# Whisper-6/DynamicTreeAttn

Measured on AMD Instinct MI355X. Metric: tree-attn fwd+bwd tokens/sec, Qwen3-0.6B tau2-16k tries, higher is better.
Workload: dtype bf16

## Files before the change

### dynamictreeattn_amd/csrc/tree_attn.hip

```cpp
#include <hip/hip_runtime.h>
#include <stdint.h>
#include <type_traits>
#include "dta_common.h"
#include "dta_device.h"

#if defined(DTA_STAMP) && DTA_STAMP
__device__ unsigned long long* dta_stamp_buf = nullptr;
extern "C" int dta_debug_set_stamp_buffer(void* p) { return hipMemcpyToSymbol(HIP_SYMBOL(dta_stamp_buf), &p, sizeof(p)) == hipSuccess ? 0 : -4; }
#define DTA_STAMP_DECL unsigned long long st_prev_, st_sum_[6] = {0, 0, 0, 0, 0, 0}; unsigned long long st_tiles_ = 0; \
  __builtin_amdgcn_sched_barrier(0); asm volatile("s_memtime %0\n\ts_waitcnt lgkmcnt(0)" : "=s"(st_prev_) :: "memory"); __builtin_amdgcn_sched_barrier(0);
#define DTA_STAMP_AT(K) { unsigned long long t_; __builtin_amdgcn_sched_barrier(0); asm volatile("s_memtime %0\n\ts_waitcnt lgkmcnt(0)" : "=s"(t_) :: "memory"); \
  __builtin_amdgcn_sched_barrier(0); st_sum_[K] += t_ - st_prev_; st_prev_ = t_; }
#define DTA_STAMP_TILE ++st_tiles_;
#define DTA_STAMP_STORE if (dta_stamp_buf && lane == 0) { unsigned long long* o_ = dta_stamp_buf + ((size_t)blockIdx.x * 8 + wave) * 8; \
  for (int k_ = 0; k_ < 6; ++k_) o_[k_] = st_sum_[k_]; o_[6] = st_tiles_; o_[7] = (unsigned long long)__builtin_amdgcn_s_getreg(0xF804) ; }
#else
#define DTA_STAMP_DECL
#define DTA_STAMP_AT(K)
#define DTA_STAMP_TILE
#define DTA_STAMP_STORE
#endif

namespace {

struct AttnParams {
  const void *q, *k, *v, *o, *dout;
  void *out, *dq, *dk, *dv;
  float *lse_w; const float* lse_r; float* delta;
  const int32_t *subtree_end, *run_ptr, *runs, *ktile_qend;
  const int32_t *dkv_units, *dkv_splits; float* dkv_ws;
  int32_t Tq, Tk, q_offset, Hq, Hkv, group;
  int32_t hgroups, head0;
  int64_t q_st, q_sh, kv_st, kv_sh, v_st, v_sh, o_st, o_sh, dq_st, dq_sh, dkv_st, dkv_sh;
  float scale; int32_t accumulate; int32_t ktile;
};
struct AttnParamsW : AttnParams { const int32_t* win_lo; int32_t window; };
struct AttnParamsC : AttnParams { float softcap; };
struct AttnParamsWC : AttnParamsW { float softcap; };
template <bool WIN, bool CAP = false> using AttnP = typename std::conditional<CAP, typename std::conditional<WIN, AttnParamsWC, AttnParamsC>::type,
                                                                              typename std::conditional<WIN, AttnParamsW, AttnParams>::type>::type;

__device__ __forceinline__ int swz64(int row) { return ((row & 2) << 1) | ((row >> 2) & 3); }
template <int D> __device__ __forceinline__ int img_off_d(int row, int ch) {
  if constexpr (D == 128) return row * 256 + ((ch ^ (((row & 3) << 2) | ((row >> 2) & 3))) << 4);
  else { static_assert(D == 64, "head_dim 64 or 128"); return row * 128 + ((ch ^ swz64(row)) << 4); }
}
template <int D> constexpr int tile_bytes() { return 64 * 2 * D; }

template <class V8, int D> __device__ __forceinline__ V8 row_frag(const char* img, int row, int ch) {
  return *reinterpret_cast<const V8*>(img + img_off_d<D>(row, ch));
}

template <class V8, int D> __device__ __forceinline__ V8 tr_frag(const char* img, int R0, int mb, int lane) {
  const int G = lane >> 4, hh = lane >> 5, i = lane & 15, qd = i >> 2, p = i & 3;
  const int ch = 4 * mb + 2 * (G & 1) + (p >> 1);
  const int ra = R0 + 4 * hh + qd;
  s16x4 lo = tr_read(img + img_off_d<D>(ra, ch) + 8 * (p & 1));
  s16x4 hi = tr_read(img + img_off_d<D>(ra + 8, ch) + 8 * (p & 1));
  s16x8 both = {lo[0], lo[1], lo[2], lo[3], hi[0], hi[1], hi[2], hi[3]};
  return __builtin_bit_cast(V8, both);
}

template <int DT> __device__ __forceinline__ typename Ty<DT>::v8 pack_half(const f32x16& x, int s2) {
  typename Ty<DT>::v8 r;
#pragma unroll
  for (int j = 0; j < 8; ++j) r[j] = (typename Ty<DT>::e)x[8 * s2 + j];
  return r;
}

__device__ __forceinline__ float fast_exp2(float x) { return __builtin_amdgcn_exp2f(x); }

#define DTA_CAP_CONSTANTS                                                                                  \
  const float c = (CAP ? cap_of(p) : p.scale) * LOG2E;                                                     \
  [[maybe_unused]] const float kcap = CAP ? 2.f * LOG2E * p.scale / cap_of(p) : 0.f;
template <class P> __device__ __forceinline__ float cap_of(const P& p) {
  if constexpr (std::is_base_of<AttnParamsC, P>::value || std::is_base_of<AttnParamsWC, P>::value) return p.softcap; else return 0.f;
}

struct TileIter {
  const int32_t* runs; int ri, re;
  int k0, kend, flag;
  int diag_first_q;
  __device__ __forceinline__ bool load_run() {
    while (ri < re) {
      k0 = __builtin_amdgcn_readfirstlane(runs[4 * ri]); kend = __builtin_amdgcn_readfirstlane(runs[4 * ri + 1]);
      flag = __builtin_amdgcn_readfirstlane(runs[4 * ri + 2]);
      if (k0 < kend) return true;
      ++ri;
    }
    return false;
  }
  __device__ __forceinline__ bool advance() {
    k0 += 64;
    if (k0 < kend) return true;
    if (runs == nullptr) return false;
    ++ri;
    return load_run();
  }
  __device__ __forceinline__ bool masked() const {
    if (runs == nullptr) return (k0 + 63 > diag_first_q) || (k0 + 64 > kend);
    return flag != 0 || (k0 + 64 > kend);
  }
};

#ifndef DTA_FWD_THR
#define DTA_FWD_THR 4.0f
#endif
constexpr float FWD_THR = DTA_FWD_THR;
constexpr int SE_BYTES = 256;

__device__ __forceinline__ float max3(float a, float b, float c) { return fmaxf(fmaxf(a, b), c); }
__device__ __forceinline__ float half_max(float x) {
  const unsigned u = __float_as_uint(x);
  const auto r = __builtin_amdgcn_permlane32_swap(u, u, false, false);
  return fmaxf(__uint_as_float(r[0]), __uint_as_float(r[1]));
}

template <int D> struct FragOffsT { int row[D / 16]; int tr[D / 16]; };
template <int D> __device__ __forceinline__ FragOffsT<D> frag_offsets(int lane) {
  FragOffsT<D> o;
  const int r = lane & 31, h = lane >> 5;
#pragma unroll
  for (int s = 0; s < D / 16; ++s) o.row[s] = img_off_d<D>(r, 2 * s + h);
  const int G = lane >> 4, i = lane & 15, qd = i >> 2, pp = i & 3;
#pragma unroll
  for (int mb = 0; mb < D / 32; ++mb) {
    const int ch = 4 * mb + 2 * (G & 1) + (pp >> 1);
    o.tr[mb] = img_off_d<D>(4 * h + qd, ch) + 8 * (pp & 1);
    o.tr[D / 32 + mb] = img_off_d<D>(4 * h + qd + 8, ch) + 8 * (pp & 1);
  }
  return o;
}
template <class V8> __device__ __forceinline__ V8 tr_pair(const char* lo_p, const char* hi_p) {
  s16x4 lo = tr_read(lo_p);
  s16x4 hi = tr_read(hi_p);
  s16x8 both = {lo[0], lo[1], lo[2], lo[3], hi[0], hi[1], hi[2], hi[3]};
  return __builtin_bit_cast(V8, both);
}
template <class V8, int D> __device__ __forceinline__ V8 tr_frag_o(const char* img_r0, const FragOffsT<D>& o, int mb) {
  s16x4 lo = tr_read(img_r0 + o.tr[mb]);
  s16x4 hi = tr_read(img_r0 + o.tr[D / 32 + mb]);
  s16x8 both = {lo[0], lo[1], lo[2], lo[3], hi[0], hi[1], hi[2], hi[3]};
  return __builtin_bit_cast(V8, both);
}

__device__ __forceinline__ uint32_t lds_addr(const void* p) {
  return (uint32_t)(uintptr_t)(__attribute__((address_space(3))) const char*)(p);
}
__device__ __forceinline__ void dma_pair2(uint32_t oa0, uint32_t oa1, const void* ba, uint32_t ob0, uint32_t ob1, const void* bb, uint32_t lds) {
  asm volatile(
      "s_nop 4\n\t"
      "s_mov_b32 m0, %6\n\t"
      "s_nop 0\n\t"
      "global_load_lds_dwordx4 %0, %4\n\t"
      "s_add_u32 m0, %6, 0x4000\n\t"
      "s_nop 0\n\t"
      "global_load_lds_dwordx4 %2, %5\n\t"
      "s_add_u32 m0, %6, 0x400\n\t"
      "s_nop 0\n\t"
      "global_load_lds_dwordx4 %1, %4\n\t"
      "s_add_u32 m0, %6, 0x4400\n\t"
// ... 39 lines not shown
      else reinterpret_cast<int*>(base_ + 2 * tile_bytes<DH>())[lane] = 0x7fffffff; }                     \
    const char* kb_ = reinterpret_cast<const char*>(kbase) + (int64_t)k0_ * p.kv_st * (int64_t)sizeof(e);  \
    const char* vb_ = reinterpret_cast<const char*>(vbase) + (int64_t)k0_ * p.v_st * (int64_t)sizeof(e);   \
    uint32_t ok_[DTA_KV_PPW(NW)], ov_[DTA_KV_PPW(NW)];                                                     \
    _Pragma("unroll") for (int i_ = 0; i_ < DTA_KV_PPW(NW); ++i_) { ok_[i_] = voff_k[i_]; ov_[i_] = voff_v[i_]; } \
    if (k0_ + 64 > p.Tk) {                          \
      _Pragma("unroll") for (int i_ = 0; i_ < DTA_KV_PPW(NW); ++i_) {                                      \
        const int row_ = DTA_KV_ROW(NW, i_);                                                               \
        const int rr_ = k0_ + row_ < p.Tk ? row_ : p.Tk - 1 - k0_;                                         \
        ok_[i_] = dma_src_off_d<DH>(rr_, row_, lane, p.kv_st, sizeof(e)); ov_[i_] = dma_src_off_d<DH>(rr_, row_, lane, p.v_st, sizeof(e)); } } \
    if constexpr (DH == 128) {                                                                             \
      _Pragma("unroll") for (int i_ = 0; i_ < DTA_KV_PPW(NW); i_ += 2)                                     \
        dma_pair2(ok_[i_], ok_[i_ + 1], kb_, ov_[i_], ov_[i_ + 1], vb_, lds_addr(base_ + (wave * DTA_KV_PPW(NW) + i_) * 1024)); \
    } else {                                                                                               \
      _Pragma("unroll") for (int i_ = 0; i_ < DTA_KV_PPW(NW); ++i_)                                        \
        dma_one2<tile_bytes<DH>()>(ok_[i_], kb_, ov_[i_], vb_, lds_addr(base_ + (wave * DTA_KV_PPW(NW) + i_) * 1024)); } }

#ifndef DTA_V_PRELOAD_N
#define DTA_V_PRELOAD_N 4
#endif
#if DTA_V_PRELOAD_N
#define DTA_V_PRELOAD v8 vpre_[DTA_V_PRELOAD_N]; _Pragma("unroll") for (int i_ = 0; i_ < DTA_V_PRELOAD_N; ++i_) { vpre_[i_] = tr_frag_o<v8>(Vs + 32 * DH * (i_ / (DH / 32)), offs, i_ % (DH / 32)); asm volatile("" : "+v"(vpre_[i_])); }
#define DTA_V_FRAG(S4, DB) (((DH / 32) * (S4) + (DB) < DTA_V_PRELOAD_N) ? vpre_[(DH / 32) * (S4) + (DB) < DTA_V_PRELOAD_N ? (DH / 32) * (S4) + (DB) : 0] : tr_frag_o<v8>(Vs + 32 * DH * (S4), offs, (DB)))
#else
#define DTA_V_PRELOAD
#define DTA_V_FRAG(S4, DB) tr_frag_o<v8>(Vs + 32 * DH * (S4), offs, (DB))
#endif

#ifndef DTA_SCORE_ORDER
#define DTA_SCORE_ORDER 1
#endif
#if DTA_SCORE_ORDER
#define DTA_SCORE_MFMAS                                                                                    \
    { v8 ka_ = *reinterpret_cast<const v8*>(Ks + offs.row[0]), kb2_ = *reinterpret_cast<const v8*>(Ks + 64 * DH + offs.row[0]); \
      _Pragma("unroll") for (int s = 0; s < DH / 16; ++s) {                                                \
        v8 na_ = ka_, nb_ = kb2_;                                                                          \
        if (s < DH / 16 - 1) { na_ = *reinterpret_cast<const v8*>(Ks + offs.row[s + 1]); nb_ = *reinterpret_cast<const v8*>(Ks + 64 * DH + offs.row[s + 1]); } \
        X[0] = T::mma(ka_, qf[s], X[0]); X[1] = T::mma(kb2_, qf[s], X[1]);                                 \
        ka_ = na_; kb2_ = nb_;                                                                             \
      } }
#else
#define DTA_SCORE_MFMAS                                                                                    \
    _Pragma("unroll") for (int kb = 0; kb < 2; ++kb)                                                       \
      _Pragma("unroll") for (int s = 0; s < DH / 16; ++s)                                                  \
        X[kb] = T::mma(*reinterpret_cast<const v8*>(Ks + 64 * DH * kb + offs.row[s]), qf[s], X[kb]);
#endif

template <int DT, int HPB, int DH, bool WIN, bool CAP>
__global__ __launch_bounds__(256 * HPB, 2) void tree_attn_fwd_kernel(AttnP<WIN, CAP> p) {
  using T = Ty<DT>; using e = typename T::e; using v8 = typename T::v8; using v4 = typename T::v4;
  constexpr int TB = tile_bytes<DH>(), NKS = DH / 16, NDB = DH / 32;
  constexpr int NW = 4 * HPB, BUF = 2 * TB + SE_BYTES;
  __shared__ __attribute__((aligned(16))) char smem[2 * BUF];

  const int tid = threadIdx.x, lane = tid & 63, r = lane & 31, h = lane >> 5;
  const int wave = __builtin_amdgcn_readfirstlane(tid >> 6);
  const int hb = wave >> 2, rw = wave & 3;
  const int bid = blockIdx.x;
  const int hgroups = p.hgroups;
  const int kvh = bid % p.Hkv; const int rest = bid / p.Hkv; const int hgb = rest % hgroups;
  const int nqt = (p.Tq + DTA_QTILE - 1) / DTA_QTILE;
  const int qt = nqt - 1 - rest / hgroups;
  const int hq = kvh * p.group + p.head0 + hgb * HPB + hb;
  const int q0 = qt * DTA_QTILE;
  const int qrow = q0 + rw * 32 + r;
  const int qrow_c = qrow < p.Tq ? qrow : p.Tq - 1;
  const int qidx = p.q_offset + qrow;
  int wlo = 0, wmax = 0;
  if constexpr (WIN) {
    wlo = p.win_lo ? p.win_lo[qrow_c] : (qidx - p.window + 1 > 0 ? qidx - p.window + 1 : 0);
    wmax = p.win_lo ? 0 : p.q_offset + (q0 + DTA_QTILE < p.Tq ? q0 + DTA_QTILE : p.Tq) - p.window;
  }

  TileIter it; it.runs = p.runs; it.diag_first_q = p.subtree_end ? -64 : p.q_offset + q0;
  if (p.runs) { it.ri = p.run_ptr[qt]; it.re = p.run_ptr[qt + 1]; if (!it.load_run()) return; }
  else { it.ri = 0; it.re = 1; it.k0 = 0; it.flag = 1; int last = p.q_offset + (q0 + DTA_QTILE < p.Tq ? q0 + DTA_QTILE : p.Tq); it.kend = last < p.Tk ? last : p.Tk; if (it.kend <= 0) return; }
  if constexpr (WIN) {
    const int lo0 = p.q_offset + q0 - p.window + 1;
    if (!p.runs && !p.win_lo && lo0 > 0) { it.k0 = lo0; if (it.k0 >= it.kend) return; }
  }

  const e* qp = reinterpret_cast<const e*>(p.q) + (int64_t)qrow_c * p.q_st + (int64_t)hq * p.q_sh;
  v8 qf[NKS];
#pragma unroll
  for (int s = 0; s < NKS; ++s) qf[s] = *reinterpret_cast<const v8*>(qp + 16 * s + 8 * h);

  const e* kbase = reinterpret_cast<const e*>(p.k) + (int64_t)kvh * p.kv_sh;
  const e* vbase = reinterpret_cast<const e*>(p.v) + (int64_t)kvh * p.v_sh;
  const FragOffsT<DH> offs = frag_offsets<DH>(lane);
  DTA_KV_OFFSETS(NW)

  f32x16 O[NDB];
#pragma unroll
  for (int db = 0; db < NDB; ++db)
#pragma unroll
    for (int g = 0; g < 16; ++g) O[db][g] = 0.f;
  float m = -1e30f, lsum = 0.f;
  DTA_CAP_CONSTANTS

  int ck0 = it.k0, ckend = it.kend; bool cmask = it.masked() || (WIN && it.k0 < wmax);
  DTA_KV_DMA(smem, it.k0, NW)
  bool has_next = it.advance();
#pragma unroll
  for (int s = 0; s < NKS; ++s) asm volatile("" : "+v"(qf[s]));
  DMA_WAIT(); __syncthreads();

#define FWD_TILE(BUFI)                                                                                     \
  {                                                                                                        \
    int nk0_ = 0, nkend_ = 0; bool nmask_ = false;                                                         \
    DTA_STAMP_AT(5) DTA_STAMP_TILE                                                                         \
    if (has_next) { nk0_ = it.k0; nkend_ = it.kend; nmask_ = it.masked() || (WIN && it.k0 < wmax); DTA_KV_DMA(smem + (1 - (BUFI)) * BUF, it.k0, NW) } \
    DTA_STAMP_AT(0)                                                                                        \
    const char* Ks = smem + (BUFI) * BUF; const char* Vs = Ks + TB;                                \
    const int* se_s = reinterpret_cast<const int*>(Ks + 2 * TB);                                   \
    f32x16 X[2];                                                                                           \
    _Pragma("unroll") for (int kb = 0; kb < 2; ++kb)                                                       \
      _Pragma("unroll") for (int g = 0; g < 16; ++g) X[kb][g] = 0.f;                                       \
    DTA_SCORE_MFMAS                                                                                        \
    if constexpr (CAP) {                          \
      _Pragma("unroll") for (int kb = 0; kb < 2; ++kb)                                                     \
        _Pragma("unroll") for (int g = 0; g < 16; ++g) X[kb][g] = cap_tanh(X[kb][g] * kcap);                 \
    }                                                                                                      \
    DTA_STAMP_AT(1)                                                                                        \
    if (cmask) {                                                                                           \
      const int qlim = qidx < ckend ? qidx : ckend - 1;       \
      _Pragma("unroll") for (int kb = 0; kb < 2; ++kb)                                                     \
        _Pragma("unroll") for (int gq = 0; gq < 4; ++gq) {                                                 \
          const int kl = 32 * kb + 8 * gq + 4 * h;                                                         \
          const int4 se4 = *reinterpret_cast<const int4*>(se_s + kl);                                      \
          const int sev[4] = {se4.x, se4.y, se4.z, se4.w};                                                 \
          _Pragma("unroll") for (int j = 0; j < 4; ++j) {                                                  \
            const bool ok = (ck0 + kl + j <= qlim) && (qidx < sev[j]) && (!WIN || ck0 + kl + j >= wlo);    \
            X[kb][4 * gq + j] = ok ? X[kb][4 * gq + j] : -INFINITY;                                        \
          }                                                                                                \
        }                                                                                                  \
    }                                                                                                      \
    DTA_V_PRELOAD                                                                                          \
    float mx = max3(X[0][0], X[0][1], X[0][2]), mx1 = max3(X[1][0], X[1][1], X[1][2]);    \
    _Pragma("unroll") for (int g = 3; g < 15; g += 2) { mx = max3(mx, X[0][g], X[0][g + 1]); mx1 = max3(mx1, X[1][g], X[1][g + 1]); } \
    mx = max3(mx, X[0][15], mx1);                                                                          \
    mx = half_max(fmaxf(mx, X[1][15]));         \
    const float mc = mx * c;                                                                               \
    if (__any(mc > m + FWD_THR)) {              \
      const float mnew = fmaxf(m, mc);                                                                     \
      const float alpha = fast_exp2(m - mnew);                                                             \
      m = mnew; lsum *= alpha;                                                                             \
      _Pragma("unroll") for (int db = 0; db < NDB; ++db)                                                   \
        _Pragma("unroll") for (int g = 0; g < 16; ++g) O[db][g] *= alpha;                                  \
    }                                                                                                      \
    DTA_STAMP_AT(2)                                                                                        \
    _Pragma("unroll") for (int kb = 0; kb < 2; ++kb)                                                       \
      _Pragma("unroll") for (int g = 0; g < 16; ++g) { const float pv = fast_exp2(__builtin_fmaf(X[kb][g], c, -m)); lsum += pv; X[kb][g] = pv; } \
    _Pragma("unroll") for (int s4 = 0; s4 < 4; ++s4) {                                                     \
      const v8 pb = pack_half<DT>(X[s4 >> 1], s4 & 1);                                                     \
      _Pragma("unroll") for (int db = 0; db < NDB; ++db) O[db] = T::mma(DTA_V_FRAG(s4, db), pb, O[db]);      \
    }                                                                                                      \
    DTA_STAMP_AT(3)                                                                                        \
    DMA_WAIT(); __syncthreads();                         \
    DTA_STAMP_AT(4)                                                                                        \
    if (!has_next) break;                                                                                  \
    ck0 = nk0_; ckend = nkend_; cmask = nmask_;                                                            \
    has_next = it.advance();                                                                               \
  }
  DTA_STAMP_DECL
  while (true) {
    FWD_TILE(0)
    FWD_TILE(1)
  }
#undef FWD_TILE
  DTA_STAMP_STORE

  lsum += __shfl_xor(lsum, 32);
  const float inv = 1.f / lsum;
  if (qrow < p.Tq) {
    e* op = reinterpret_cast<e*>(p.out) + (int64_t)qrow * p.o_st + (int64_t)hq * p.o_sh;
#pragma unroll
    for (int db = 0; db < NDB; ++db)
#pragma unroll
      for (int gq = 0; gq < 4; ++gq) {
        v4 w;
#pragma unroll
        for (int j = 0; j < 4; ++j) w[j] = (e)(O[db][4 * gq + j] * inv);
        *reinterpret_cast<v4*>(op + 32 * db + 8 * gq + 4 * h) = w;
      }
    if (h == 0) p.lse_w[(int64_t)hq * p.Tq + qrow] = m + __builtin_amdgcn_logf(lsum);
  }
}

template <int DT, int HPB, int DH, bool WIN, bool CAP>
__global__ __launch_bounds__(256 * HPB, 2) void tree_attn_bwd_dq_kernel(AttnP<WIN, CAP> p) {
  using T = Ty<DT>; using e = typename T::e; using v8 = typename T::v8; using v4 = typename T::v4;
  constexpr int TB = tile_bytes<DH>(), NKS = DH / 16, NDB = DH / 32;
  __shared__ __attribute__((aligned(16))) char smem[2 * (2 * TB + SE_BYTES)];

  const int tid = threadIdx.x, lane = tid & 63, r = lane & 31, h = lane >> 5;
  const int wave = __builtin_amdgcn_readfirstlane(tid >> 6);
  const int hb = wave >> 2, rw = wave & 3;
  const int bid = blockIdx.x;
  const int hgroups = p.hgroups;
  const int kvh = bid % p.Hkv; const int rest = bid / p.Hkv; const int hgb = rest % hgroups;
  const int nqt = (p.Tq + DTA_QTILE - 1) / DTA_QTILE;
  const int qt = nqt - 1 - rest / hgroups;
  const int hq = kvh * p.group + p.head0 + hgb * HPB + hb;
  const int q0 = qt * DTA_QTILE;
  const int qrow = q0 + rw * 32 + r;
  const int qrow_c = qrow < p.Tq ? qrow : p.Tq - 1;
  const int qidx = p.q_offset + qrow;
  int wlo = 0, wmax = 0;
  if constexpr (WIN) {
    wlo = p.win_lo ? p.win_lo[qrow_c] : (qidx - p.window + 1 > 0 ? qidx - p.window + 1 : 0);
    wmax = p.win_lo ? 0 : p.q_offset + (q0 + DTA_QTILE < p.Tq ? q0 + DTA_QTILE : p.Tq) - p.window;
  }

  const e* qp = reinterpret_cast<const e*>(p.q) + (int64_t)qrow_c * p.q_st + (int64_t)hq * p.q_sh;
  const e* dop = reinterpret_cast<const e*>(p.dout) + (int64_t)qrow_c * p.o_st + (int64_t)hq * p.o_sh;
  const e* op = reinterpret_cast<const e*>(p.o) + (int64_t)qrow_c * p.o_st + (int64_t)hq * p.o_sh;
  v8 qf[NKS], dof[NKS];
  float dsum = 0.f;
#pragma unroll
  for (int s = 0; s < NKS; ++s) {
    qf[s] = *reinterpret_cast<const v8*>(qp + 16 * s + 8 * h);
    dof[s] = *reinterpret_cast<const v8*>(dop + 16 * s + 8 * h);
    const v8 of = *reinterpret_cast<const v8*>(op + 16 * s + 8 * h);
#pragma unroll
    for (int j = 0; j < 8; ++j) dsum += (float)dof[s][j] * (float)of[j];
  }
  dsum += __shfl_xor(dsum, 32);
  const float delta = dsum;
  const float lse2 = p.lse_r[(int64_t)hq * p.Tq + qrow_c];
  if (h == 0 && qrow < p.Tq) p.delta[(int64_t)hq * p.Tq + qrow] = -delta;

  TileIter it; it.runs = p.runs; it.diag_first_q = p.subtree_end ? -64 : p.q_offset + q0;
  bool any = true;
  if (p.runs) { it.ri = p.run_ptr[qt]; it.re = p.run_ptr[qt + 1]; any = it.load_run(); }
  else { it.ri = 0; it.re = 1; it.k0 = 0; it.flag = 1; int last = p.q_offset + (q0 + DTA_QTILE < p.Tq ? q0 + DTA_QTILE : p.Tq); it.kend = last < p.Tk ? last : p.Tk; any = it.kend > 0; }
  if constexpr (WIN) {
    const int lo0 = p.q_offset + q0 - p.window + 1;
    if (!p.runs && !p.win_lo && lo0 > 0) { it.k0 = lo0; any = any && it.k0 < it.kend; }
  }

  const e* kbase = reinterpret_cast<const e*>(p.k) + (int64_t)kvh * p.kv_sh;
  const e* vbase = reinterpret_cast<const e*>(p.v) + (int64_t)kvh * p.v_sh;
  constexpr int NW = 4 * HPB, BUF = 2 * TB + SE_BYTES;
  DTA_KV_OFFSETS(NW)

  f32x16 DQ[NDB];
#pragma unroll
  for (int db = 0; db < NDB; ++db)
#pragma unroll
    for (int g = 0; g < 16; ++g) DQ[db][g] = 0.f;
  DTA_CAP_CONSTANTS

  f32x16 DI;
#pragma unroll
  for (int g = 0; g < 16; ++g) DI[g] = -delta;
  if (any) {
    int ck0 = it.k0, ckend = it.kend; bool cmask = it.masked() || (WIN && it.k0 < wmax);
    DTA_KV_DMA(smem, it.k0, NW)
    bool has_next = it.advance();
    DMA_WAIT(); __syncthreads();
    int cur = 0;
    while (true) {
      int nk0 = 0, nkend = 0; bool nmask = false;
      if (has_next) { nk0 = it.k0; nkend = it.kend; nmask = it.masked() || (WIN && it.k0 < wmax); DTA_KV_DMA(smem + (cur ^ 1) * BUF, it.k0, NW) }
      const char* Ks = smem + cur * BUF; const char* Vs = Ks + TB;
      const int* se_s = reinterpret_cast<const int*>(Ks + 2 * TB);
#pragma unroll
      for (int kb = 0; kb < 2; ++kb) {
        f32x16 X, DP;
#pragma unroll
        for (int g = 0; g < 16; ++g) X[g] = 0.f;
        {
          v8 kf_ = row_frag<v8, DH>(Ks, 32 * kb + r, h), vf_ = row_frag<v8, DH>(Vs, 32 * kb + r, h);
#pragma unroll
          for (int s = 0; s < NKS; ++s) {
            v8 nk_ = kf_, nv_ = vf_;
            if (s < NKS - 1) { nk_ = row_frag<v8, DH>(Ks, 32 * kb + r, 2 * s + 2 + h); nv_ = row_frag<v8, DH>(Vs, 32 * kb + r, 2 * s + 2 + h); }
            X = T::mma(kf_, qf[s], X);
            DP = T::mma(vf_, dof[s], s == 0 ? DI : DP);
            kf_ = nk_; vf_ = nv_;
          }
          __builtin_amdgcn_sched_group_barrier(0x100, 4, 0);
#pragma unroll
          for (int i_ = 0; i_ < NKS - 2; ++i_) { __builtin_amdgcn_sched_group_barrier(0x008, 2, 0); __builtin_amdgcn_sched_group_barrier(0x100, 2, 0); }
          __builtin_amdgcn_sched_group_barrier(0x008, 4, 0);
        }
        if (cmask) {
          const int qlim = qidx < ckend ? qidx : ckend - 1;
#pragma unroll
          for (int gq = 0; gq < 4; ++gq) {
            const int kl = 32 * kb + 8 * gq + 4 * h;
            const int4 se4 = *reinterpret_cast<const int4*>(se_s + kl);
            const int sev[4] = {se4.x, se4.y, se4.z, se4.w};
#pragma unroll
            for (int j = 0; j < 4; ++j) {
              const int g = 4 * gq + j;
              const bool ok = (ck0 + kl + j <= qlim) && (qidx < sev[j]) && (!WIN || ck0 + kl + j >= wlo);
              if constexpr (CAP) {
                const float t = cap_tanh(X[g] * kcap);
                const float pv = ok ? fast_exp2(__builtin_fmaf(t, c, -lse2)) : 0.f;
                X[g] = pv * DP[g] * __builtin_fmaf(-t, t, 1.f);
              } else {
              const float pv = ok ? fast_exp2(__builtin_fmaf(X[g], c, -lse2)) : 0.f;
              X[g] = pv * DP[g];
              }
            }
          }
        } else {
#pragma unroll
          for (int g = 0; g < 16; ++g) {
            if constexpr (CAP) { const float t = cap_tanh(X[g] * kcap); X[g] = fast_exp2(__builtin_fmaf(t, c, -lse2)) * DP[g] * __builtin_fmaf(-t, t, 1.f); }
            else X[g] = fast_exp2(__builtin_fmaf(X[g], c, -lse2)) * DP[g];
          }
        }
#pragma unroll
        for (int s2 = 0; s2 < 2; ++s2) {
          const v8 db_ = pack_half<DT>(X, s2);
#pragma unroll
          for (int db = 0; db < NDB; ++db) DQ[db] = T::mma(tr_frag<v8, DH>(Ks, 32 * kb + 16 * s2, db, lane), db_, DQ[db]);
        }
      }
      DMA_WAIT(); __syncthreads();
      if (!has_next) break;
      cur ^= 1; ck0 = nk0; ckend = nkend; cmask = nmask;
      has_next = it.advance();
    }
  }
  if (qrow < p.Tq) {
    e* dqp = reinterpret_cast<e*>(p.dq) + (int64_t)qrow * p.dq_st + (int64_t)hq * p.dq_sh;
#pragma unroll
    for (int db = 0; db < NDB; ++db)
#pragma unroll
      for (int gq = 0; gq < 4; ++gq) {
        v4 w;
#pragma unroll
        for (int j = 0; j < 4; ++j) w[j] = (e)(DQ[db][4 * gq + j] * p.scale);
        *reinterpret_cast<v4*>(dqp + 32 * db + 8 * gq + 4 * h) = w;
      }
  }
}

#ifndef DTA_KV2_PIN
#define DTA_KV2_PIN 2
#endif
#if DTA_KV2_PIN == 2
#define DTA_KV2_PIN_ORDER                                                                                  \
    __builtin_amdgcn_sched_group_barrier(0x100, 4, 0);                                                     \
    _Pragma("unroll") for (int i_ = 0; i_ < 2 * NKS; ++i_) { __builtin_amdgcn_sched_group_barrier(0x100, 2, 0); __builtin_amdgcn_sched_group_barrier(0x008, 1, 0); }
#elif DTA_KV2_PIN
#define DTA_KV2_PIN_ORDER                                                                                  \
    __builtin_amdgcn_sched_group_barrier(0x100, 12, 0);                                                    \
    _Pragma("unroll") for (int i_ = 0; i_ < NKS - 2; ++i_) { __builtin_amdgcn_sched_group_barrier(0x008, 2, 0); __builtin_amdgcn_sched_group_barrier(0x100, 4, 0); } \
    __builtin_amdgcn_sched_group_barrier(0x008, 4, 0);
#else
#define DTA_KV2_PIN_ORDER
#endif

template <int D> constexpr int kv2_slot() { return 2 * (D / 16) * 1024; }
template <int D> constexpr int kv2_frags() { return 4 * kv2_slot<D>(); }
template <int D, bool WIN> constexpr int kv2_buf() { return 2 * tile_bytes<D>() + (WIN ? 768 : 512); }
template <int D, bool WIN> constexpr int kv2_lds() { return kv2_frags<D>() + 2 * kv2_buf<D, WIN>() + 16; }

template <int DT, int DH, bool WIN, bool CAP>
__global__ __launch_bounds__(512, 2) void tree_attn_bwd_dkv2_kernel(AttnP<WIN, CAP> p) {
  using T = Ty<DT>; using e = typename T::e; using v8 = typename T::v8; using v4 = typename T::v4;
  constexpr int KT = 128;
  constexpr int TB = tile_bytes<DH>(), NKS = DH / 16, NDB = DH / 32, KV2_FRAGS = kv2_frags<DH>(), KV2_BUF = kv2_buf<DH, WIN>(), KSLOT = kv2_slot<DH>();
  __shared__ __attribute__((aligned(16))) char smem_all[kv2_lds<DH, WIN>()];
  const int tid8 = threadIdx.x, tid = tid8 & 255, lane = tid & 63, r = lane & 31, h = lane >> 5;
  const int wave8 = __builtin_amdgcn_readfirstlane(tid8 >> 6);
  const int grp = wave8 >> 2, wave = wave8 & 3;
  char* kvs = smem_all + wave * KSLOT;
  char* smem = smem_all + KV2_FRAGS;
  const int bid = blockIdx.x;
  const int kvh = bid % p.Hkv; const int unit = bid / p.Hkv;
  const int kt = p.dkv_units ? p.dkv_units[4 * unit] : unit;
  const int slab = p.dkv_units ? p.dkv_units[4 * unit + 3] : -1;
  const int k0 = kt * KT;
  const int q_hi = p.q_offset + p.Tq;
  const int kidx = k0 + wave * 32 + r;
  int se_l;
  { const int kc = kidx < p.Tk ? kidx : p.Tk - 1;
    int se = (kidx < p.Tk) ? (p.subtree_end ? p.subtree_end[kidx] : 0x7fffffff) : 0;
    se_l = se < q_hi ? se : q_hi;
    if (grp == 0) {
      const e* kp = reinterpret_cast<const e*>(p.k) + (int64_t)kc * p.kv_st + (int64_t)kvh * p.kv_sh;
      const e* vp = reinterpret_cast<const e*>(p.v) + (int64_t)kc * p.v_st + (int64_t)kvh * p.v_sh;
#pragma unroll
      for (int s = 0; s < NKS; ++s) {
        *reinterpret_cast<v8*>(kvs + s * 1024 + lane * 16) = *reinterpret_cast<const v8*>(kp + 16 * s + 8 * h);
        *reinterpret_cast<v8*>(kvs + KSLOT / 2 + s * 1024 + lane * 16) = *reinterpret_cast<const v8*>(vp + 16 * s + 8 * h);
      }
    } }
  int* se_min_s = reinterpret_cast<int*>(smem_all + KV2_FRAGS + 2 * KV2_BUF);
  { int mn = se_l;
#pragma unroll
    for (int o = 32; o > 0; o >>= 1) { const int t = __shfl_xor(mn, o); mn = t < mn ? t : mn; }
    if (lane == 0 && grp == 0) se_min_s[wave] = mn; }
  __syncthreads();
  const int se_min = __builtin_amdgcn_readfirstlane(min(min(se_min_s[0], se_min_s[1]), min(se_min_s[2], se_min_s[3])));

  const FragOffsT<DH> offs = frag_offsets<DH>(lane);
  f32x16 DK[NDB], DV[NDB];
#pragma unroll
  for (int db = 0; db < NDB; ++db)
#pragma unroll
    for (int g = 0; g < 16; ++g) { DK[db][g] = 0.f; DV[db][g] = 0.f; }

  int qbeg, qend;
  if (p.dkv_units) { qbeg = __builtin_amdgcn_readfirstlane(p.dkv_units[4 * unit + 1]); qend = __builtin_amdgcn_readfirstlane(p.dkv_units[4 * unit + 2]); }
  else {
    qbeg = k0 > p.q_offset ? k0 : p.q_offset;
    qend = p.ktile_qend ? p.ktile_qend[kt] : q_hi; qend = qend < q_hi ? qend : q_hi;
    if constexpr (WIN) if (!p.win_lo) {
      const int64_t wl = (int64_t)k0 + KT - 1 + p.window; qend = wl < qend ? (int)wl : qend;
    }
  }
  const int ntile = qend > qbeg ? (qend - qbeg + 63) / 64 : 0;
  const int total = ntile * p.group;
  DTA_CAP_CONSTANTS

// ... 58 lines not shown
      const v8 ad = *reinterpret_cast<const v8*>(tb + ar[s] + TB);                                         \
      const v8 kfs = *reinterpret_cast<const v8*>(kvs + s * 1024 + lane * 16);                             \
      const v8 vfs = *reinterpret_cast<const v8*>(kvs + KSLOT / 2 + s * 1024 + lane * 16);                 \
      S = T::mma(aq, kfs, S); DP = T::mma(ad, vfs, DP);                                                    \
    }                                                                                                      \
    DTA_KV2_PIN_ORDER                                                                                      \
    float nl[16];                                                                                          \
    _Pragma("unroll") for (int gq = 0; gq < 4; ++gq) {                                                     \
      const float4 l4 = *reinterpret_cast<const float4*>(rc + 32 * gq);                                    \
      nl[4 * gq] = l4.x; nl[4 * gq + 1] = l4.y; nl[4 * gq + 2] = l4.z; nl[4 * gq + 3] = l4.w;              \
    }                                                                                                      \
    if constexpr (CAP) {                            \
      _Pragma("unroll") for (int g = 0; g < 16; ++g) { const float t = cap_tanh(S[g] * kcap); S[g] = t; DP[g] *= __builtin_fmaf(-t, t, 1.f); } \
    }                                                                                                      \
    if (full) {                                                                                            \
      _Pragma("unroll") for (int g = 0; g < 16; ++g) {                                                     \
        const float pv = fast_exp2(__builtin_fmaf(S[g], c, -nl[g]));                                       \
        S[g] = pv;                                                                                         \
        DP[g] = pv * DP[g];                                                                                \
      }                                                                                                    \
    } else {                                                                                               \
      int wl[16];                                    \
      if constexpr (WIN) {                                                                                 \
        if (p.win_lo) {                                                                                    \
          _Pragma("unroll") for (int gq = 0; gq < 4; ++gq) {                                               \
            const int4 w4 = *reinterpret_cast<const int4*>(rc + 512 + 32 * gq);                            \
            wl[4 * gq] = w4.x; wl[4 * gq + 1] = w4.y; wl[4 * gq + 2] = w4.z; wl[4 * gq + 3] = w4.w; }      \
        } else {                                                                                           \
          _Pragma("unroll") for (int g = 0; g < 16; ++g) wl[g] = qi0 + 8 * (g >> 2) + 4 * h + (g & 3) - p.window + 1; } \
      }                                                                                                    \
      _Pragma("unroll") for (int g = 0; g < 16; ++g) {                                                     \
        const int qi = qi0 + 8 * (g >> 2) + 4 * h + (g & 3);                                               \
        const bool ok = (kidx <= qi) && (qi < se_l) && (!WIN || kidx >= wl[g]);                            \
        const float pv = ok ? fast_exp2(__builtin_fmaf(S[g], c, -nl[g])) : 0.f;                            \
        S[g] = pv;                                                                                         \
        DP[g] = pv * DP[g];                                                                                \
      }                                                                                                    \
    }                                                                                                      \
    _Pragma("unroll") for (int s2 = 0; s2 < 2; ++s2) {                                                     \
      const v8 pb = pack_half<DT>(S, s2), sbf = pack_half<DT>(DP, s2);                                     \
      _Pragma("unroll") for (int db = 0; db < NDB; ++db) {                                                 \
        const v8 adt = tr_pair<v8>(tb + at[db] + TB + 32 * DH * s2, tb + at[NDB + db] + TB + 32 * DH * s2); \
        const v8 aqt = tr_pair<v8>(tb + at[db] + 32 * DH * s2, tb + at[NDB + db] + 32 * DH * s2);          \
        DV[db] = T::mma(adt, pb, DV[db]); DK[db] = T::mma(aqt, sbf, DK[db]);                               \
      }                                                                                                    \
    }                                                                                                      \
    DMA_WAIT(); __syncthreads();                                                                           \
    ++idx;                                                                                                 \
  }

  {
    int ti_c = 0;
    if (total > 0) KV2_DMA(0)
    DMA_WAIT(); __syncthreads();
    int idx = 0;
    while (idx < total) {
      KV2_TILE(0)
      if (idx >= total) break;
      KV2_TILE(1)
    }
  }
#undef KV2_TILE
#undef KV2_DMA
  {
    float* red = reinterpret_cast<float*>(smem_all);
#pragma unroll
    for (int db = 0; db < NDB; ++db) {
      if (grp == 1) {
#pragma unroll
        for (int g = 0; g < 16; ++g) { red[g * 256 + tid] = DK[db][g]; red[(16 + g) * 256 + tid] = DV[db][g]; }
      }
      __syncthreads();
      if (grp == 0) {
#pragma unroll
        for (int g = 0; g < 16; ++g) { DK[db][g] += red[g * 256 + tid]; DV[db][g] += red[(16 + g) * 256 + tid]; }
      }
      __syncthreads();
    }
    if (grp == 1) return;
  }
#pragma unroll
  for (int db = 0; db < NDB; ++db)
#pragma unroll
    for (int g = 0; g < 16; ++g) DK[db][g] *= p.scale;
  const int kloc = wave * 32 + r;
  if (slab >= 0) {
    float* ws = p.dkv_ws + ((int64_t)slab * p.Hkv + kvh) * (2 * KT * DH) + (int64_t)kloc * DH;
#pragma unroll
    for (int db = 0; db < NDB; ++db)
#pragma unroll
      for (int gq = 0; gq < 4; ++gq) {
        const int d = 32 * db + 8 * gq + 4 * h;
        *reinterpret_cast<float4*>(ws + d) = make_float4(DK[db][4 * gq], DK[db][4 * gq + 1], DK[db][4 * gq + 2], DK[db][4 * gq + 3]);
        *reinterpret_cast<float4*>(ws + KT * DH + d) = make_float4(DV[db][4 * gq], DV[db][4 * gq + 1], DV[db][4 * gq + 2], DV[db][4 * gq + 3]);
      }
  } else if (kidx < p.Tk && p.accumulate == 2) {
    float* dkp = reinterpret_cast<float*>(p.dk) + (int64_t)kidx * p.dkv_st + (int64_t)kvh * p.dkv_sh;
    float* dvp = reinterpret_cast<float*>(p.dv) + (int64_t)kidx * p.dkv_st + (int64_t)kvh * p.dkv_sh;
#pragma unroll
    for (int db = 0; db < NDB; ++db)
#pragma unroll
      for (int gq = 0; gq < 4; ++gq) {
        const int d = 32 * db + 8 * gq + 4 * h;
        float4 a = *reinterpret_cast<const float4*>(dkp + d), b = *reinterpret_cast<const float4*>(dvp + d);
        a.x += DK[db][4 * gq]; a.y += DK[db][4 * gq + 1]; a.z += DK[db][4 * gq + 2]; a.w += DK[db][4 * gq + 3];
        b.x += DV[db][4 * gq]; b.y += DV[db][4 * gq + 1]; b.z += DV[db][4 * gq + 2]; b.w += DV[db][4 * gq + 3];
        *reinterpret_cast<float4*>(dkp + d) = a;
        *reinterpret_cast<float4*>(dvp + d) = b;
      }
  } else if (kidx < p.Tk) {
    e* dkp = reinterpret_cast<e*>(p.dk) + (int64_t)kidx * p.dkv_st + (int64_t)kvh * p.dkv_sh;
    e* dvp = reinterpret_cast<e*>(p.dv) + (int64_t)kidx * p.dkv_st + (int64_t)kvh * p.dkv_sh;
#pragma unroll
    for (int db = 0; db < NDB; ++db)
#pragma unroll
      for (int gq = 0; gq < 4; ++gq) {
        const int d = 32 * db + 8 * gq + 4 * h;
        v4 wk, wv;
        if (p.accumulate) {
          const v4 ok_ = *reinterpret_cast<const v4*>(dkp + d); const v4 ov_ = *reinterpret_cast<const v4*>(dvp + d);
#pragma unroll
          for (int j = 0; j < 4; ++j) { wk[j] = (e)(DK[db][4 * gq + j] + (float)ok_[j]); wv[j] = (e)(DV[db][4 * gq + j] + (float)ov_[j]); }
        } else {
#pragma unroll
          for (int j = 0; j < 4; ++j) { wk[j] = (e)DK[db][4 * gq + j]; wv[j] = (e)DV[db][4 * gq + j]; }
        }
        *reinterpret_cast<v4*>(dkp + d) = wk;
        *reinterpret_cast<v4*>(dvp + d) = wv;
      }
  }
}

constexpr int FIN_SPLIT = 8;
template <int DT, int DH>
__global__ __launch_bounds__(256) void tree_attn_bwd_dkv_finalize_kernel(AttnParams p) {
  using e = typename Ty<DT>::e; using v4 = typename Ty<DT>::v4;
  const int KT = p.ktile;
  const int kvh = blockIdx.x % p.Hkv, sp = blockIdx.x / p.Hkv;
  const int kt = p.dkv_splits[4 * sp], first = p.dkv_splits[4 * sp + 1], n = p.dkv_splits[4 * sp + 2];
  constexpr int Q4 = DH / 4, Q4_SHIFT = DH == 128 ? 5 : 4;
  const int per = 2 * KT * Q4 / FIN_SPLIT;
  const float* ws0 = p.dkv_ws + ((int64_t)first * p.Hkv + kvh) * (2 * KT * DH);
  const int64_t slab_st = (int64_t)p.Hkv * (2 * KT * DH);
  for (int i = blockIdx.y * per + threadIdx.x; i < (blockIdx.y + 1) * per; i += 256) {
    const int which = i / (KT * Q4), rem = i - which * KT * Q4;
    const int key = rem >> Q4_SHIFT, d = (rem & (Q4 - 1)) << 2;
    const int kidx = kt * KT + key;
    if (kidx >= p.Tk) continue;
    float4 acc = make_float4(0.f, 0.f, 0.f, 0.f);
    int j = 0;
    for (; j + 4 <= n; j += 4) {
      const float4 a0 = *reinterpret_cast<const float4*>(ws0 + (j + 0) * slab_st + (int64_t)i * 4);
      const float4 a1 = *reinterpret_cast<const float4*>(ws0 + (j + 1) * slab_st + (int64_t)i * 4);
      const float4 a2 = *reinterpret_cast<const float4*>(ws0 + (j + 2) * slab_st + (int64_t)i * 4);
      const float4 a3 = *reinterpret_cast<const float4*>(ws0 + (j + 3) * slab_st + (int64_t)i * 4);
      acc.x += a0.x; acc.y += a0.y; acc.z += a0.z; acc.w += a0.w;
      acc.x += a1.x; acc.y += a1.y; acc.z += a1.z; acc.w += a1.w;
      acc.x += a2.x; acc.y += a2.y; acc.z += a2.z; acc.w += a2.w;
      acc.x += a3.x; acc.y += a3.y; acc.z += a3.z; acc.w += a3.w;
    }
    for (; j < n; ++j) {
      const float4 v = *reinterpret_cast<const float4*>(ws0 + j * slab_st + (int64_t)i * 4);
      acc.x += v.x; acc.y += v.y; acc.z += v.z; acc.w += v.w;
    }
    if (p.accumulate == 2) {
      float* outf = reinterpret_cast<float*>(which ? p.dv : p.dk) + (int64_t)kidx * p.dkv_st + (int64_t)kvh * p.dkv_sh + d;
      float4 o = *reinterpret_cast<const float4*>(outf);
      o.x += acc.x; o.y += acc.y; o.z += acc.z; o.w += acc.w;
      *reinterpret_cast<float4*>(outf) = o;
      continue;
    }
    e* out = reinterpret_cast<e*>(which ? p.dv : p.dk) + (int64_t)kidx * p.dkv_st + (int64_t)kvh * p.dkv_sh + d;
    if (p.accumulate) { const v4 o = *reinterpret_cast<const v4*>(out); acc.x += (float)o[0]; acc.y += (float)o[1]; acc.z += (float)o[2]; acc.w += (float)o[3]; }
    v4 w; w[0] = (e)acc.x; w[1] = (e)acc.y; w[2] = (e)acc.z; w[3] = (e)acc.w;
    *reinterpret_cast<v4*>(out) = w;
  }
}

template <bool WIN, bool CAP> AttnP<WIN, CAP> kernel_params(const DtaAttnArgs& a) {
  AttnP<WIN, CAP> p{};
  if constexpr (WIN) { p.win_lo = a.win_lo; p.window = a.window; }
  if constexpr (CAP) p.softcap = a.softcap;
  p.q = a.q; p.k = a.k; p.v = a.v; p.o = a.o; p.dout = a.dout; p.out = a.out; p.dq = a.dq; p.dk = a.dk; p.dv = a.dv;
// ... 128 lines not shown
```

Baseline: 858,800.

## Stage epilogue outputs through swizzled LDS for coalesced row stores; halve dkv reduction rounds

The forward O, backward dQ and dK/dV epilogues now write each wave's fragment into a swizzled LDS staging area, then read it back so that each lane stores full 16-byte row chunks to global memory. This replaces scattered 8-byte per-lane stores with coalesced writes. The dK/dV cross-group reduction now moves half the head dimension per round, which needs fewer LDS round-trips and barriers. Optional seam timestamp instrumentation is added under a debug macro. The cost is extra LDS traffic and a wait in the epilogue, and correctness depends on the staging regions not overlapping data other waves still need.

```diff
diff --git a/dynamictreeattn_amd/csrc/tree_attn.hip b/dynamictreeattn_amd/csrc/tree_attn.hip
--- a/dynamictreeattn_amd/csrc/tree_attn.hip
+++ b/dynamictreeattn_amd/csrc/tree_attn.hip
@@ -7,6 +7,18 @@
 #if defined(DTA_STAMP) && DTA_STAMP
 __device__ unsigned long long* dta_stamp_buf = nullptr;
 extern "C" int dta_debug_set_stamp_buffer(void* p) { return hipMemcpyToSymbol(HIP_SYMBOL(dta_stamp_buf), &p, sizeof(p)) == hipSuccess ? 0 : -4; }
+#endif
+#if defined(DTA_STAMP) && DTA_STAMP == 2
+#define DTA_SEAM_DECL unsigned long long seam_[4] = {0, 0, 0, 0};
+#define DTA_SEAM_AT(K) { __builtin_amdgcn_sched_barrier(0); asm volatile("s_memtime %0\n\ts_waitcnt lgkmcnt(0)" : "=s"(seam_[K]) :: "memory"); __builtin_amdgcn_sched_barrier(0); }
+#define DTA_SEAM_STORE(W, KID) { asm volatile("s_waitcnt vmcnt(0)" ::: "memory"); DTA_SEAM_AT(3)  \
+  if (dta_stamp_buf && (W) == 0 && lane == 0 && blockIdx.x < 65536) { unsigned long long* o_ = dta_stamp_buf + ((size_t)(KID) * 65536 + blockIdx.x) * 4; for (int k_ = 0; k_ < 4; ++k_) o_[k_] = seam_[k_]; } }
+#else
+#define DTA_SEAM_DECL
+#define DTA_SEAM_AT(K)
+#define DTA_SEAM_STORE(W, KID)
+#endif
+#if defined(DTA_STAMP) && DTA_STAMP == 1
 #define DTA_STAMP_DECL unsigned long long st_prev_, st_sum_[6] = {0, 0, 0, 0, 0, 0}; unsigned long long st_tiles_ = 0; \
   __builtin_amdgcn_sched_barrier(0); asm volatile("s_memtime %0\n\ts_waitcnt lgkmcnt(0)" : "=s"(st_prev_) :: "memory"); __builtin_amdgcn_sched_barrier(0);
 #define DTA_STAMP_AT(K) { unsigned long long t_; __builtin_amdgcn_sched_barrier(0); asm volatile("s_memtime %0\n\ts_waitcnt lgkmcnt(0)" : "=s"(t_) :: "memory"); \
@@ -107,6 +119,35 @@
 #define DTA_FWD_THR 4.0f
 #endif
 constexpr float FWD_THR = DTA_FWD_THR;
+
+template <int D> __device__ __forceinline__ int stage_off(int r, int c) {
+  if constexpr (D == 128) return (c ^ (r & 15)) << 4;
+  else return ((r & 1) << 7) | ((c ^ ((r >> 1) & 7)) << 4);
+}
+template <int DT, int D, int NDB> __device__ __forceinline__ void stage_row(char* slot, int r, int h, const f32x16 (&A)[NDB], float mul) {
+  using e = typename Ty<DT>::e; using v4 = typename Ty<DT>::v4;
+#pragma unroll
+  for (int db = 0; db < NDB; ++db)
+#pragma unroll
+    for (int gq = 0; gq < 4; ++gq) {
+      v4 w;
+#pragma unroll
+      for (int j = 0; j < 4; ++j) w[j] = (e)(A[db][4 * gq + j] * mul);
+      *reinterpret_cast<v4*>(slot + stage_off<D>(r, 4 * db + gq) + 8 * h) = w;
+    }
+}
+template <int DT, int D> __device__ __forceinline__ void store_rows(const char* stage, int pitch, typename Ty<DT>::e* g, int64_t stride, int row0, int nrows, int lane) {
+  using v8 = typename Ty<DT>::v8;
+  constexpr int CPR = D / 8, RPI = 64 / CPR;
+  asm volatile("s_waitcnt lgkmcnt(0)" ::: "memory");
+  const int c = lane & (CPR - 1), rl = lane / CPR;
+#pragma unroll
+  for (int i = 0; i < 32 / RPI; ++i) {
+    const int ri = RPI * i + rl;
+    const v8 w = *reinterpret_cast<const v8*>(stage + (D == 128 ? ri : ri >> 1) * pitch + stage_off<D>(ri, c));
+    if (row0 + ri < nrows) *reinterpret_cast<v8*>(g + (int64_t)(row0 + ri) * stride + 8 * c) = w;
+  }
+}
 constexpr int SE_BYTES = 256;
 
 __device__ __forceinline__ float max3(float a, float b, float c) { return fmaxf(fmaxf(a, b), c); }
@@ -252,6 +293,7 @@
   constexpr int TB = tile_bytes<DH>(), NKS = DH / 16, NDB = DH / 32;
   constexpr int NW = 4 * HPB, BUF = 2 * TB + SE_BYTES;
   __shared__ __attribute__((aligned(16))) char smem[2 * BUF];
+  DTA_SEAM_DECL DTA_SEAM_AT(0)
 
   const int tid = threadIdx.x, lane = tid & 63, r = lane & 31, h = lane >> 5;
   const int wave = __builtin_amdgcn_readfirstlane(tid >> 6);
@@ -303,7 +345,7 @@
   bool has_next = it.advance();
 #pragma unroll
   for (int s = 0; s < NKS; ++s) asm volatile("" : "+v"(qf[s]));
-  DMA_WAIT(); __syncthreads();
+  DMA_WAIT(); __syncthreads(); DTA_SEAM_AT(1)
 
 #define FWD_TILE(BUFI)                                                                                     \
   {                                                                                                        \
@@ -368,23 +410,18 @@
     FWD_TILE(1)
   }
 #undef FWD_TILE
+  DTA_SEAM_AT(2)
   DTA_STAMP_STORE
 
   lsum += __shfl_xor(lsum, 32);
   const float inv = 1.f / lsum;
-  if (qrow < p.Tq) {
-    e* op = reinterpret_cast<e*>(p.out) + (int64_t)qrow * p.o_st + (int64_t)hq * p.o_sh;
-#pragma unroll
-    for (int db = 0; db < NDB; ++db)
-#pragma unroll
-      for (int gq = 0; gq < 4; ++gq) {
-        v4 w;
-#pragma unroll
-        for (int j = 0; j < 4; ++j) w[j] = (e)(O[db][4 * gq + j] * inv);
-        *reinterpret_cast<v4*>(op + 32 * db + 8 * gq + 4 * h) = w;
-      }
-    if (h == 0) p.lse_w[(int64_t)hq * p.Tq + qrow] = m + __builtin_amdgcn_logf(lsum);
-  }
+  {
+    char* stage = smem + wave * (64 * DH);
+    stage_row<DT, DH, NDB>(stage + (DH == 128 ? r : r >> 1) * 256, r, h, O, inv);
+    store_rows<DT, DH>(stage, 256, reinterpret_cast<e*>(p.out) + (int64_t)hq * p.o_sh, p.o_st, q0 + rw * 32, p.Tq, lane);
+    if (h == 0 && qrow < p.Tq) p.lse_w[(int64_t)hq * p.Tq + qrow] = m + __builtin_amdgcn_logf(lsum);
+  }
+  DTA_SEAM_STORE(wave, 0)
 }
 
 template <int DT, int HPB, int DH, bool WIN, bool CAP>
@@ -392,6 +429,7 @@
   using T = Ty<DT>; using e = typename T::e; using v8 = typename T::v8; using v4 = typename T::v4;
   constexpr int TB = tile_bytes<DH>(), NKS = DH / 16, NDB = DH / 32;
   __shared__ __attribute__((aligned(16))) char smem[2 * (2 * TB + SE_BYTES)];
+  DTA_SEAM_DECL DTA_SEAM_AT(0)
 
   const int tid = threadIdx.x, lane = tid & 63, r = lane & 31, h = lane >> 5;
   const int wave = __builtin_amdgcn_readfirstlane(tid >> 6);
@@ -458,7 +496,7 @@
     int ck0 = it.k0, ckend = it.kend; bool cmask = it.masked() || (WIN && it.k0 < wmax);
     DTA_KV_DMA(smem, it.k0, NW)
     bool has_next = it.advance();
-    DMA_WAIT(); __syncthreads();
+    DMA_WAIT(); __syncthreads(); DTA_SEAM_AT(1)
     int cur = 0;
     while (true) {
       int nk0 = 0, nkend = 0; bool nmask = false;
@@ -526,18 +564,13 @@
       has_next = it.advance();
     }
   }
-  if (qrow < p.Tq) {
-    e* dqp = reinterpret_cast<e*>(p.dq) + (int64_t)qrow * p.dq_st + (int64_t)hq * p.dq_sh;
-#pragma unroll
-    for (int db = 0; db < NDB; ++db)
-#pragma unroll
-      for (int gq = 0; gq < 4; ++gq) {
-        v4 w;
-#pragma unroll
-        for (int j = 0; j < 4; ++j) w[j] = (e)(DQ[db][4 * gq + j] * p.scale);
-        *reinterpret_cast<v4*>(dqp + 32 * db + 8 * gq + 4 * h) = w;
-      }
-  }
+  DTA_SEAM_AT(2)
+  {
+    char* stage = smem + wave * (64 * DH);
+    stage_row<DT, DH, NDB>(stage + (DH == 128 ? r : r >> 1) * 256, r, h, DQ, p.scale);
+    store_rows<DT, DH>(stage, 256, reinterpret_cast<e*>(p.dq) + (int64_t)hq * p.dq_sh, p.dq_st, q0 + rw * 32, p.Tq, lane);
+  }
+  DTA_SEAM_STORE(wave, 1)
 }
 
 #ifndef DTA_KV2_PIN
@@ -567,6 +600,7 @@
   constexpr int KT = 128;
   constexpr int TB = tile_bytes<DH>(), NKS = DH / 16, NDB = DH / 32, KV2_FRAGS = kv2_frags<DH>(), KV2_BUF = kv2_buf<DH, WIN>(), KSLOT = kv2_slot<DH>();
   __shared__ __attribute__((aligned(16))) char smem_all[kv2_lds<DH, WIN>()];
+  DTA_SEAM_DECL DTA_SEAM_AT(0)
   const int tid8 = threadIdx.x, tid = tid8 & 255, lane = tid & 63, r = lane & 31, h = lane >> 5;
   const int wave8 = __builtin_amdgcn_readfirstlane(tid8 >> 6);
   const int grp = wave8 >> 2, wave = wave8 & 3;
@@ -731,7 +765,7 @@
   {
     int ti_c = 0;
     if (total > 0) KV2_DMA(0)
-    DMA_WAIT(); __syncthreads();
+    DMA_WAIT(); __syncthreads(); DTA_SEAM_AT(1)
     int idx = 0;
     while (idx < total) {
       KV2_TILE(0)
@@ -739,22 +773,28 @@
       KV2_TILE(1)
     }
   }
+  DTA_SEAM_AT(2)
 #undef KV2_TILE
 #undef KV2_DMA
   {
+    static_assert(kv2_lds<DH, WIN>() >= NDB * 16 * 256 * 4, "a hand-off round must fit the kernel's LDS");
     float* red = reinterpret_cast<float*>(smem_all);
 #pragma unroll
-    for (int db = 0; db < NDB; ++db) {
+    for (int hf = 0; hf < 2; ++hf) {
       if (grp == 1) {
 #pragma unroll
-        for (int g = 0; g < 16; ++g) { red[g * 256 + tid] = DK[db][g]; red[(16 + g) * 256 + tid] = DV[db][g]; }
+        for (int db = 0; db < NDB / 2; ++db)
+#pragma unroll
+          for (int g = 0; g < 16; ++g) { red[(32 * db + g) * 256 + tid] = DK[hf * (NDB / 2) + db][g]; red[(32 * db + 16 + g) * 256 + tid] = DV[hf * (NDB / 2) + db][g]; }
       }
       __syncthreads();
       if (grp == 0) {
 #pragma unroll
-        for (int g = 0; g < 16; ++g) { DK[db][g] += red[g * 256 + tid]; DV[db][g] += red[(16 + g) * 256 + tid]; }
+        for (int db = 0; db < NDB / 2; ++db)
+#pragma unroll
+          for (int g = 0; g < 16; ++g) { DK[hf * (NDB / 2) + db][g] += red[(32 * db + g) * 256 + tid]; DV[hf * (NDB / 2) + db][g] += red[(32 * db + 16 + g) * 256 + tid]; }
       }
-      __syncthreads();
+      if (hf == 0) __syncthreads();
     }
     if (grp == 1) return;
   }
@@ -773,6 +813,14 @@
         *reinterpret_cast<float4*>(ws + d) = make_float4(DK[db][4 * gq], DK[db][4 * gq + 1], DK[db][4 * gq + 2], DK[db][4 * gq + 3]);
         *reinterpret_cast<float4*>(ws + KT * DH + d) = make_float4(DV[db][4 * gq], DV[db][4 * gq + 1], DV[db][4 * gq + 2], DV[db][4 * gq + 3]);
       }
+  } else if (p.accumulate == 0) {
+    constexpr int NSLOT = DH / 4;
+    char* stage = smem_all + wave * 256;
+    const int slot = (DH == 128 ? r : r >> 1) * 1024;
+    stage_row<DT, DH, NDB>(stage + slot, r, h, DK, 1.f);
+    stage_row<DT, DH, NDB>(stage + NSLOT * 1024 + slot, r, h, DV, 1.f);
+    store_rows<DT, DH>(stage, 1024, reinterpret_cast<e*>(p.dk) + (int64_t)kvh * p.dkv_sh, p.dkv_st, k0 + wave * 32, p.Tk, lane);
+    store_rows<DT, DH>(stage + NSLOT * 1024, 1024, reinterpret_cast<e*>(p.dv) + (int64_t)kvh * p.dkv_sh, p.dkv_st, k0 + wave * 32, p.Tk, lane);
   } else if (kidx < p.Tk && p.accumulate == 2) {
     float* dkp = reinterpret_cast<float*>(p.dk) + (int64_t)kidx * p.dkv_st + (int64_t)kvh * p.dkv_sh;
     float* dvp = reinterpret_cast<float*>(p.dv) + (int64_t)kidx * p.dkv_st + (int64_t)kvh * p.dkv_sh;
@@ -808,6 +856,7 @@
         *reinterpret_cast<v4*>(dvp + d) = wv;
       }
   }
+  DTA_SEAM_STORE(wave8, 2)
 }
 
 constexpr int FIN_SPLIT = 8;
```

Result: no change. 862,300, median of 5 (+0.4%).
